# SNUCP/MKHE-KKLSS

Measured on AMD Instinct MI355X. Metric: mkckks_mulrelin_per_sec, higher is better.
Workload: dtype u64; 1 GPU; mkckks 4-party MulRelin (hoist + MulAndRelinHoisted + Rescale), PN15QP880 N=2^15, 14 Q + 2 P limbs; parties=4, params=PN15QP880, seed=1296779333, key_material=host

## Files before the change

### mkhe-kklss_amd/csrc/ntt_kernels.hip

```cpp
#include "ntt_kernels.h"
#include <stdexcept>
#include <cstdlib>
#include <mutex>
#ifndef MKHE_SB_MASK
#define MKHE_SB_MASK 1
#endif
#ifndef MKHE_TW_CHUNK
#define MKHE_TW_CHUNK 4
#endif

namespace mkhe {

typedef const __attribute__((address_space(1))) u64* gcptr;
typedef __attribute__((address_space(1))) u64* gptr;

template <int LOGN> struct Geo {
    static constexpr int N = 1 << LOGN;
    static constexpr int T = N / 32;
    static constexpr int BT = T < 64 ? 64 : T;
    static constexpr int LPB = BT / T;
    static constexpr int MIDTOP = (LOGN - 6) < 9 ? (LOGN - 6) : 9;
    static constexpr int MIDB = MIDTOP - 5;
    static constexpr bool HAS_MID = MIDTOP >= 5;
};
// ... 68 lines not shown
    if constexpr (!CROSS) lds_sync<false>();
}

__device__ __forceinline__ void bfly_fwd_cs(u64& U, u64& V, u64 ws, u64 q, u64 q2, u64 qs, u32 ninv) {
    u64 Tm = mont_mul_sdu(V, ws, qs, q, ninv);
    u64 u = csub(U, q2);
    U = u + Tm;
    V = u + (q2 - Tm);
}
__device__ __forceinline__ void bfly_fwd_nr(u64& U, u64& V, u64 ws, u64 qs, u32 ninv) {
    const i64 Tm = mont_mul_sd((i64)V, ws, qs, ninv);
    const i64 u = (i64)U;
    U = (u64)(u + Tm);
    V = (u64)(u - Tm);
}
__device__ __forceinline__ void bfly_inv(u64& U, u64& V, u64 ws, u64 q, u64 q2, u64 qs, u32 ninv) {
    u64 s = csub(U + V, q2);
    u64 d = U + q2 - V;
    U = s;
    V = mont_mul_sdu(d, ws, qs, q, ninv);
}

template <int B, int MODE>
__device__ __forceinline__ void stage(u64 (&x)[32], gcptr tw, u64 q, u64 q2, u64 qs, u32 ninv) {
    constexpr int NW = 16 >> B;
#ifdef MKHE_NO_CHUNK
    constexpr int CH = NW;
#else
    constexpr int CH = NW < MKHE_TW_CHUNK ? NW : MKHE_TW_CHUNK;
#endif
    constexpr int NCH = NW / CH;
    constexpr int BPC = 16 / NCH;
    u64 wc[CH], wn[CH];
#pragma unroll
    for (int k = 0; k < CH; ++k) wc[k] = tw[k];
#pragma unroll
    for (int c = 0; c < NCH; ++c) {
        if (c + 1 < NCH) {
#pragma unroll
            for (int k = 0; k < CH; ++k) wn[k] = tw[(c + 1) * CH + k];
        }
#pragma unroll
        for (int gg = 0; gg < BPC; ++gg) {
            const int g = c * BPC + gg;
            const int i0 = ((g >> B) << (B + 1)) | (g & ((1 << B) - 1));
            const int i1 = i0 | (1 << B);
            const u64 w = wc[(g >> B) - c * CH];
            if constexpr (MODE == 2) bfly_inv(x[i0], x[i1], w, q, q2, qs, ninv);
            else if constexpr (MODE == 1) bfly_fwd_nr(x[i0], x[i1], w, qs, ninv);
            else bfly_fwd_cs(x[i0], x[i1], w, q, q2, qs, ninv);
#ifndef MKHE_NO_SCHEDBAR
            if ((gg & MKHE_SB_MASK) == MKHE_SB_MASK) __builtin_amdgcn_sched_barrier(0);
#endif
        }
        if (c + 1 < NCH) {
#pragma unroll
            for (int k = 0; k < CH; ++k) wc[k] = wn[k];
        }
    }
    asm volatile("" ::: "memory");
}

template <int MODE>
__device__ __forceinline__ void phase(u64 (&x)[32], gcptr psi, int base, int prefix, int maxB, u64 q, u64 q2, u64 qs, u32 ninv) {
    if constexpr (MODE != 2) {
        if (maxB >= 4) stage<4, MODE>(x, psi + (base >> 4) + prefix, q, q2, qs, ninv);
        if (maxB >= 3) stage<3, MODE>(x, psi + (base >> 3) + (prefix << 1), q, q2, qs, ninv);
        if (maxB >= 2) stage<2, MODE>(x, psi + (base >> 2) + (prefix << 2), q, q2, qs, ninv);
        if (maxB >= 1) stage<1, MODE>(x, psi + (base >> 1) + (prefix << 3), q, q2, qs, ninv);
        if (maxB >= 0) stage<0, MODE>(x, psi + base + (prefix << 4), q, q2, qs, ninv);
    } else {
        if (maxB >= 0) stage<0, MODE>(x, psi + base + (prefix << 4), q, q2, qs, ninv);
        if (maxB >= 1) stage<1, MODE>(x, psi + (base >> 1) + (prefix << 3), q, q2, qs, ninv);
        if (maxB >= 2) stage<2, MODE>(x, psi + (base >> 2) + (prefix << 2), q, q2, qs, ninv);
        if (maxB >= 3) stage<3, MODE>(x, psi + (base >> 3) + (prefix << 1), q, q2, qs, ninv);
        if (maxB >= 4) stage<4, MODE>(x, psi + (base >> 4) + prefix, q, q2, qs, ninv);
    }
}

typedef const __attribute__((address_space(4))) NttBatch* kargptr;
__device__ __forceinline__ unsigned vi_parts_of(kargptr kb, int item) {
    return (((const __attribute__((address_space(4))) unsigned*)kb->vi_parts)[item >> 1] >> (16 * (item & 1))) & 0xffffu;
}
template <bool VI = false>
__device__ __forceinline__ int job_pointers(const NttBatch& b, int job, gcptr& src, gptr& dst, int& m, int& outer, int* pm = nullptr) {
    kargptr kb = (kargptr)__builtin_amdgcn_kernarg_segment_ptr();
    const int s = job / b.nouter;
    outer = job - s * b.nouter;
    m = kb->mod[s];
    if (VI && b.vi) {
        const int cnt = kb->vi_cnt[outer];
        const int k = s < b.vi_q ? 0 : (s - b.vi_q) / b.vi_np;
        const bool exists = k < cnt;
        const unsigned mem = kb->vi_mem[outer];
        const int item = (int)((mem >> (exists ? 8 * k : 0)) & 255u);
        const long off = (long)item * b.src_outer + (long)m * b.src_inner;
        src = (gcptr)(b.src + off);
        dst = (gptr)(b.dst + off);
        if (pm) *pm = s < b.vi_q ? -1 : k;
        if (!exists) return 0;
        if (s >= b.vi_q) return 1 + (int)(vi_parts_of(kb, item) & 255u);
        int n = kb->vi_extra[outer] != nullptr ? 1 : 0;
        for (int j = 0; j < cnt; ++j) n += 1 + (int)(vi_parts_of(kb, (mem >> (8 * j)) & 255u) & 255u);
        return n;
    }
    if (pm) *pm = -1;
    const int p = kb->pos[s];
    const u64* sbase = b.src; u64* dbase = b.dst;
    if (b.nitems > 0) {
        const int item = outer / b.outers_per_item;
        outer -= item * b.outers_per_item;
        sbase = kb->src_items[item]; dbase = kb->dst_items[item];
    }
    src = (gcptr)(sbase + (long)outer * b.src_outer + (long)(b.src_mapped ? m : p) * b.src_inner);
    dst = (gptr)(dbase + (long)outer * b.dst_outer + (long)(b.dst_mapped ? m : p) * b.dst_inner);
    return 1;
}
__device__ __forceinline__ long vi_member_offset(const NttBatch& b, int g, int k, int m, gcptr first) {
    kargptr kb = (kargptr)__builtin_amdgcn_kernarg_segment_ptr();
    if (k >= kb->vi_cnt[g]) return (long)(((u64)kb->vi_extra[g] - (u64)first) >> 3) + (long)m * b.src_inner;
    const unsigned mem = kb->vi_mem[g];
    return ((long)((mem >> (8 * k)) & 255u) - (long)(mem & 255u)) * b.src_outer;
}
__device__ __forceinline__ long vi_summand_offset(const NttBatch& b, int g, int pm, int k, int m, gcptr first) {
    kargptr kb = (kargptr)__builtin_amdgcn_kernarg_segment_ptr();
    const unsigned mem = kb->vi_mem[g];
    if (pm >= 0) {
        const int item = (int)((mem >> (8 * pm)) & 255u);
        return ((long)(vi_parts_of(kb, item) >> 8) + (k - 1) - (long)item) * b.src_outer;
    }
    const int cnt = kb->vi_cnt[g], item0 = (int)(mem & 255u);
    int kk = k;
    for (int j = 0; j < cnt; ++j) {
        const int item = (int)((mem >> (8 * j)) & 255u);
        const unsigned parts = vi_parts_of(kb, item);
        const int np_ = 1 + (int)(parts & 255u);
        if (kk < np_) return ((long)(kk == 0 ? item : (int)(parts >> 8) + kk - 1) - (long)item0) * b.src_outer;
        kk -= np_;
    }
    return (long)(((u64)kb->vi_extra[g] - (u64)first) >> 3) + (long)m * b.src_inner;
}

#ifdef MKHE_PHASE_TRACE
#define MKHE_STAMP(k) do { if (b.trace && (threadIdx.x & 63) == 0 && active) b.trace[((long)job * 16 + (threadIdx.x >> 6)) * 16 + (k)] = __builtin_amdgcn_s_memtime(); } while (0)
#else
#define MKHE_STAMP(k) do { } while (0)
#endif
template <int LOGN, int MODE, bool DEC>
__device__ __forceinline__ void ntt_fwd_job(const NttBatch& b, int job, bool active, u32* lds, int t) {
    using G = Geo<LOGN>;
#ifdef MKHE_PHASE_TRACE
    if (b.trace && (threadIdx.x & 63) == 0 && active) {
        u64* tw = b.trace + ((long)job * 16 + (threadIdx.x >> 6)) * 16;
        tw[12] = __builtin_amdgcn_s_memrealtime();
        tw[14] = __builtin_amdgcn_s_getreg((4 << 0) | (0 << 6) | (31 << 11));
    }
#endif
    MKHE_STAMP(0);
    gcptr src; gptr dst; int m, outer;
    const int half = b.split ? (job & 1) : 0;
    job_pointers(b, b.split ? (job >> 1) : job, src, dst, m, outer);
    src += half * G::N; dst += half * G::N;
    const int root = b.split ? 2 + half : 1;
    const Mod md = b.mods[m];
    const u64 q = md.q, q2 = md.q2;
    const u32 ninv = md.ninv32;
    gcptr psi = (gcptr)(b.psi + ((long)m * G::N << b.split));

    u64 x[32];
#pragma unroll
    for (int r = 0; r < 32; ++r) x[r] = src[posA<LOGN>(t, r)];
#ifdef MKHE_PHASE_TRACE
    if (b.trace) { asm volatile("s_waitcnt vmcnt(0)" ::: "memory"); MKHE_STAMP(1); }
#endif
    if constexpr (DEC) {
        int sm = m;
        if (b.reduce_src_mod_is_outer == 1) sm = outer;
        else if (b.reduce_src_mod_is_outer == 2) sm = ((kargptr)__builtin_amdgcn_kernarg_segment_ptr())->outer_mod[outer];
        const u64 qs = b.mods[sm].q << (b.src_lazy ? 2 : 0);
        if (qs > 4 * q) {
#pragma unroll
            for (int r = 0; r < 32; ++r) {
                if constexpr (MODE == 1) x[r] = (u64)mont_mul_sd((i64)x[r], md.r1s, md.qs, ninv);
                else x[r] = mont_mul_sdu(x[r], md.r1s, md.qs, q, ninv);
            }
        }
    }
#pragma unroll 1
    for (int ph = 0; ph < 3; ++ph) {
        int base = 16, prefix = 0, maxB = 4;
        if (ph == 1) { base = G::N >> 6; prefix = t >> 5; maxB = G::MIDB; }
        if (ph == 2) { base = G::N >> 1; prefix = t; }
        phase<MODE>(x, psi, base * root, prefix, maxB, q, q2, md.qs, ninv);
        MKHE_STAMP(2 + 2 * ph);
        if (ph == 0) {
            if constexpr (G::HAS_MID) {
                __syncthreads();
                exchange<LOGN, LA, LB, true>(x, lds, t);
            }
        } else if (ph == 1) exchange<LOGN, LB, LC, false>(x, lds, t);
        MKHE_STAMP(3 + 2 * ph);
    }
    if constexpr (MODE == 1) {
        if (!b.skip_norm) {
#pragma unroll
            for (int r = 0; r < 32; ++r) {
                const i64 y = mont_mul_sd((i64)x[r], md.r1s, md.qs, ninv);
                x[r] = (u64)(y + ((y >> 63) & (i64)q));
            }
        } else {
            const i64 bias = (i64)(q << 4);
#pragma unroll
            for (int r = 0; r < 32; ++r) x[r] = (u64)((i64)x[r] + bias);
        }
    } else {
#pragma unroll
        for (int r = 0; r < 32; ++r) x[r] = csub(csub(x[r], q2), q);
    }
    MKHE_STAMP(7);
    exchange<LOGN, LC, LB, false>(x, lds, t);
    MKHE_STAMP(8);
    if (active) {
#pragma unroll
// ... 82 lines not shown
        phase<2>(x, psi, base * root, prefix, maxB, q, q2, md.qs, ninv);
        if (ph == 0) exchange_xor<LOGN, LC, LB, false>(x, lds, t);
        else { if constexpr (G::HAS_MID) exchange_xor<LOGN, LB, LA, true>(x, lds, t); }
    }
    phase<2>(x, psi, 16 * root, 0, 3, q, q2, md.qs, ninv);
    const int ax = 6 * m + (b.split ? 2 + 2 * half : 0);
    const u64 ninvR = b.aux[ax], w1n = b.aux[ax + 1];
#pragma unroll
    for (int g = 0; g < 16; ++g) {
        u64 U = x[g], V = x[g + 16];
        u64 s = mont_mul_sdu(U + V, ninvR, md.qs, q, ninv);
        u64 d = mont_mul_sdu(U + q2 - V, w1n, md.qs, q, ninv);
        x[g] = (b.lazy_out | b.split) ? s : csub(s, q);
        x[g + 16] = (b.lazy_out | b.split) ? d : csub(d, q);
    }
    if (exists) {
#pragma unroll
        for (int r = 0; r < 32; ++r) dst[posA<LOGN>(t, r)] = x[r];
    }
    }
}

constexpr int SPLIT_THREADS = 256;
template <bool DEC>
__global__ void __launch_bounds__(SPLIT_THREADS) ntt_split_fwd_kernel(NttBatch b, int logN) {
    const int N = 1 << logN, H = N >> 1;
    gcptr src; gptr dst; int m, outer;
    job_pointers(b, blockIdx.y, src, dst, m, outer);
    const Mod md = b.mods[m];
    const u64 q = md.q, q2 = md.q2;
    const u32 ninv = md.ninv32;
    const u64 w = b.psi[(long)m * N + 1];
    bool red = false;
    if constexpr (DEC) {
        int sm = m;
        if (b.reduce_src_mod_is_outer == 1) sm = outer;
        else if (b.reduce_src_mod_is_outer == 2) sm = ((kargptr)__builtin_amdgcn_kernarg_segment_ptr())->outer_mod[outer];
        const u64 qs = b.mods[sm].q << (b.src_lazy ? 2 : 0);
        red = qs > 4 * q;
    }
    for (int j = blockIdx.x * SPLIT_THREADS + threadIdx.x; j < H; j += gridDim.x * SPLIT_THREADS) {
        u64 U = src[j], V = src[j + H];
        if (red) { U = mont_mul_sdu(U, md.r1s, md.qs, q, ninv); V = mont_mul_sdu(V, md.r1s, md.qs, q, ninv); }
        else U = csub(U, q2);
        const u64 Tm = mont_mul_sdu(V, w, md.qs, q, ninv);
        dst[j] = U + Tm;
        dst[j + H] = U + (q2 - Tm);
    }
}
__global__ void __launch_bounds__(SPLIT_THREADS) ntt_split_inv_kernel(NttBatch b, int logN) {
    const int N = 1 << logN, H = N >> 1;
    gcptr src; gptr dst; int m, outer;
    if (!job_pointers<true>(b, blockIdx.y, src, dst, m, outer)) return;
    const Mod md = b.mods[m];
    const u64 q = md.q, q2 = md.q2;
    const u32 ninv = md.ninv32;
    const u64 w = b.psi[(long)m * N + 1];
    for (int j = blockIdx.x * SPLIT_THREADS + threadIdx.x; j < H; j += gridDim.x * SPLIT_THREADS) {
        const u64 U = dst[j], V = dst[j + H];
        u64 s = csub(U + V, q2);
        u64 d = mont_mul_sdu(U + q2 - V, w, md.qs, q, ninv);
        if (!b.lazy_out) { s = csub(s, q); d = csub(d, q); }
        dst[j] = s;
        dst[j + H] = d;
    }
}
constexpr int SM_LOGM = 13, SM_M = 1 << SM_LOGM, SM_T = 1024, SM_E = SM_M / SM_T;
constexpr int SM_LDS_WORDS = SM_M + (SM_M >> 3);
__device__ __forceinline__ int sm_pad(int p) { return p + ((p >> 4) << 1); }

template <int LOGM> struct SmGeo { static constexpr int T = LOGM == 11 ? 256 : LOGM == 12 ? 512 : SM_T, E = (1 << LOGM) / T, LDSW = (1 << LOGM) + (1 << (LOGM - 3)); };
template <int S0, int NB, int LOGM>
__device__ __forceinline__ void sm_tw_load(gcptr psi, int root, int t, u64* tw) {
    constexpr int LGL = LOGM - S0 - NB, UPT = SmGeo<LOGM>::E >> NB, NE = 1 << NB;
#pragma unroll
    for (int k = 0; k < UPT; ++k) {
        const int high = (k * SmGeo<LOGM>::T + t) >> LGL;
#pragma unroll
        for (int i = 0; i < NB; ++i)
#pragma unroll
            for (int j = 0; j < (1 << i); ++j) tw[k * (NE - 1) + (1 << i) - 1 + j] = psi[(root << (S0 + i)) + (high << i) + j];
    }
}
template <int S0, int NB, bool FROM_G, bool TO_G, int MODE, int FIN, int LOGM = SM_LOGM, bool PRE = false>
__device__ __forceinline__ void sm_phase(gcptr gsrc, gptr gdst, u64* lds, gcptr psi, int root, int t, const Mod& md, u64 fin_c, int skip_norm,
                                         int nsum = 1, const long* sum_off = nullptr, const u64* tw = nullptr) {
    constexpr int LGL = LOGM - S0 - NB, GL = 1 << LGL, UPT = SmGeo<LOGM>::E >> NB, NE = 1 << NB;
    const u64 q = md.q, q2 = md.q2;
    const u32 ninv = md.ninv32;
#pragma unroll
    for (int k = 0; k < UPT; ++k) {
        const int u = k * SmGeo<LOGM>::T + t;
        const int low = u & (GL - 1), high = u >> LGL;
        const int p = (high << (LGL + NB)) | low;
        u64 x[NE];
#pragma unroll
        for (int a = 0; a < NE; ++a) x[a] = FROM_G ? gsrc[p + a * GL] : lds[sm_pad(p + a * GL)];
        if constexpr (FROM_G && MODE == 2) {
#pragma unroll
            for (int k = 1; k < VI_SUMS; ++k)
                if (k < nsum) {
#pragma unroll
                    for (int a = 0; a < NE; ++a) x[a] = csub(x[a] + gsrc[sum_off[k] + p + a * GL], q);
                }
        }
#pragma unroll
        for (int ii = 0; ii < NB; ++ii) {
            const int i = MODE == 2 ? NB - 1 - ii : ii;
            const int half = 1 << (NB - 1 - i);
#pragma unroll
            for (int a = 0; a < NE; ++a) {
                if (a & half) continue;
                const u64 w = PRE ? tw[k * (NE - 1) + (1 << i) - 1 + (a >> (NB - i))] : psi[(root << (S0 + i)) + (high << i) + (a >> (NB - i))];
                if constexpr (MODE == 2) bfly_inv(x[a], x[a + half], w, q, q2, md.qs, ninv);
                else if constexpr (MODE == 1) bfly_fwd_nr(x[a], x[a + half], w, md.qs, ninv);
                else bfly_fwd_cs(x[a], x[a + half], w, q, q2, md.qs, ninv);
            }
        }
#pragma unroll
        for (int a = 0; a < NE; ++a) {
            u64 v = x[a];
            if constexpr (FIN == 1) {
                if constexpr (MODE == 1) {
                    if (!skip_norm) { const i64 y = mont_mul_sd((i64)v, md.r1s, md.qs, ninv); v = (u64)(y + ((y >> 63) & (i64)q)); }
                    else v = (u64)((i64)v + (i64)(q << 4));
                } else v = csub(csub(v, q2), q);
            } else if constexpr (FIN == 2) v = mont_mul_sdu(v, fin_c, md.qs, q, ninv);
            if constexpr (TO_G) gdst[p + a * GL] = v; else lds[sm_pad(p + a * GL)] = v;
        }
    }
}

template <int MODE, int LOGM = SM_LOGM>
__global__ void __launch_bounds__(SmGeo<LOGM>::T) ntt_fwd_lds_kernel(NttBatch b, int d) {
    extern __shared__ __attribute__((aligned(16))) u64 sm_lds[];
    constexpr int M = 1 << LOGM;
    const int job = blockIdx.x, part = job & ((1 << d) - 1), t = threadIdx.x;
    gcptr src; gptr dst; int m, outer;
    job_pointers(b, job >> d, src, dst, m, outer);
    src += part * M; dst += part * M;
    const int root = (1 << d) + part;
    const Mod md = b.mods[m];
    gcptr psi = (gcptr)(b.psi + ((long)m * M << d));
    if constexpr (LOGM <= 12) {
        constexpr int NBL = LOGM == 12 ? 3 : 2, NL = (SmGeo<LOGM>::E >> NBL) * ((1 << NBL) - 1);
        u64 t0[7], t1[7], t2[7], t3[NL];
        sm_tw_load<0, 3, LOGM>(psi, root, t, t0); sm_tw_load<3, 3, LOGM>(psi, root, t, t1);
        sm_tw_load<6, 3, LOGM>(psi, root, t, t2); sm_tw_load<9, NBL, LOGM>(psi, root, t, t3);
        sm_phase<0, 3, true, false, MODE, 0, LOGM, true>(src, dst, sm_lds, psi, root, t, md, 0, 0, 1, nullptr, t0);
        __syncthreads();
        sm_phase<3, 3, false, false, MODE, 0, LOGM, true>(src, dst, sm_lds, psi, root, t, md, 0, 0, 1, nullptr, t1);
        __syncthreads();
        sm_phase<6, 3, false, false, MODE, 0, LOGM, true>(src, dst, sm_lds, psi, root, t, md, 0, 0, 1, nullptr, t2);
        __syncthreads();
        sm_phase<9, NBL, false, true, MODE, 1, LOGM, true>(src, dst, sm_lds, psi, root, t, md, 0, b.skip_norm, 1, nullptr, t3);
    } else {
        sm_phase<0, 3, true, false, MODE, 0, LOGM>(src, dst, sm_lds, psi, root, t, md, 0, 0);
        __syncthreads();
        sm_phase<3, 3, false, false, MODE, 0, LOGM>(src, dst, sm_lds, psi, root, t, md, 0, 0);
        __syncthreads();
        sm_phase<6, 3, false, false, MODE, 0, LOGM>(src, dst, sm_lds, psi, root, t, md, 0, 0);
        __syncthreads();
        sm_phase<9, 3, false, false, MODE, 0, LOGM>(src, dst, sm_lds, psi, root, t, md, 0, 0);
        __syncthreads();
        sm_phase<12, 1, false, true, MODE, 1, LOGM>(src, dst, sm_lds, psi, root, t, md, 0, b.skip_norm);
    }
}

template <int LOGM>
__global__ void __launch_bounds__(SmGeo<LOGM>::T) ntt_inv_ldsS_kernel(NttBatch b, int d) {
    extern __shared__ __attribute__((aligned(16))) u64 sm_lds[];
    constexpr int M = 1 << LOGM;
    const int job = blockIdx.x, part = job & ((1 << d) - 1), t = threadIdx.x;
    gcptr src; gptr dst; int m, outer;
    int pm = -1;
    const int nsum = job_pointers<true>(b, job >> d, src, dst, m, outer, &pm);
    if (nsum == 0) return;
    long sum_off[VI_SUMS] = {};
#pragma unroll
    for (int k = 1; k < VI_SUMS; ++k) if (k < nsum) sum_off[k] = vi_summand_offset(b, outer, pm, k, m, src);
    src += part * M; dst += part * M;
    const int root = (1 << d) + part;
    const Mod md = b.mods[m];
    gcptr psi = (gcptr)(b.psi + ((long)m * M << d));
    const u64 ninvR = b.aux[6 * m];
    constexpr int NBL = LOGM == 12 ? 3 : 2, NL = (SmGeo<LOGM>::E >> NBL) * ((1 << NBL) - 1);
    u64 t0[7], t1[7], t2[7], t3[NL];
    sm_tw_load<9, NBL, LOGM>(psi, root, t, t3); sm_tw_load<6, 3, LOGM>(psi, root, t, t2);
    sm_tw_load<3, 3, LOGM>(psi, root, t, t1); sm_tw_load<0, 3, LOGM>(psi, root, t, t0);
    sm_phase<9, NBL, true, false, 2, 0, LOGM, true>(src, dst, sm_lds, psi, root, t, md, 0, 0, nsum, sum_off, t3);
    __syncthreads();
    sm_phase<6, 3, false, false, 2, 0, LOGM, true>(src, dst, sm_lds, psi, root, t, md, 0, 0, 1, nullptr, t2);
    __syncthreads();
    sm_phase<3, 3, false, false, 2, 0, LOGM, true>(src, dst, sm_lds, psi, root, t, md, 0, 0, 1, nullptr, t1);
    __syncthreads();
    sm_phase<0, 3, false, true, 2, 2, LOGM, true>(src, dst, sm_lds, psi, root, t, md, ninvR, 0, 1, nullptr, t0);
}

__global__ void __launch_bounds__(SPLIT_THREADS) ntt_pass_fwd_kernel(NttBatch b, int logN, int L) {
    const int N = 1 << logN, G = N >> (L + 1);
    gcptr src; gptr dst; int m, outer;
    job_pointers(b, blockIdx.y, src, dst, m, outer);
    const Mod md = b.mods[m];
    const u64 q = md.q, q2 = md.q2;
    const u32 ninv = md.ninv32;
    for (int j = blockIdx.x * SPLIT_THREADS + threadIdx.x; j < (N >> 1); j += gridDim.x * SPLIT_THREADS) {
        const int blk = j >> (logN - L - 1), off = j - blk * G, i0 = blk * 2 * G + off;
        const u64 w = b.psi[(long)m * N + (1 << L) + blk];
        const u64 U = csub(dst[i0], q2), V = dst[i0 + G];
        const u64 Tm = mont_mul_sdu(V, w, md.qs, q, ninv);
        dst[i0] = U + Tm;
        dst[i0 + G] = U + (q2 - Tm);
    }
}
__global__ void __launch_bounds__(SPLIT_THREADS) ntt_pass_inv_kernel(NttBatch b, int logN, int L) {
    const int N = 1 << logN, G = N >> (L + 1);
    gcptr src; gptr dst; int m, outer;
    if (!job_pointers<true>(b, blockIdx.y, src, dst, m, outer)) return;
    const Mod md = b.mods[m];
    const u64 q = md.q, q2 = md.q2;
    const u32 ninv = md.ninv32;
    for (int j = blockIdx.x * SPLIT_THREADS + threadIdx.x; j < (N >> 1); j += gridDim.x * SPLIT_THREADS) {
        const int blk = j >> (logN - L - 1), off = j - blk * G, i0 = blk * 2 * G + off;
        const u64 w = b.psi[(long)m * N + (1 << L) + blk];
        const u64 U = dst[i0], V = dst[i0 + G];
        dst[i0] = csub(U + V, q2);
        dst[i0 + G] = mont_mul_sdu(U + q2 - V, w, md.qs, q, ninv);
    }
}

template <bool DEC>
__global__ void __launch_bounds__(SPLIT_THREADS) ntt_pass4_fwd_kernel(NttBatch b, int logN) {
    const int N = 1 << logN, Q = N >> 2;
    gcptr src; gptr dst; int m, outer;
    job_pointers(b, blockIdx.y, src, dst, m, outer);
    const Mod md = b.mods[m];
    const u64 q = md.q, q2 = md.q2;
    const u32 ninv = md.ninv32;
    const u64 w1 = b.psi[(long)m * N + 1], w2 = b.psi[(long)m * N + 2], w3 = b.psi[(long)m * N + 3];
    bool red = false;
    if constexpr (DEC) {
        int sm = m;
        if (b.reduce_src_mod_is_outer == 1) sm = outer;
        else if (b.reduce_src_mod_is_outer == 2) sm = ((kargptr)__builtin_amdgcn_kernarg_segment_ptr())->outer_mod[outer];
        const u64 qs = b.mods[sm].q << (b.src_lazy ? 2 : 0);
        red = qs > 4 * q;
    }
    for (int j = blockIdx.x * SPLIT_THREADS + threadIdx.x; j < Q; j += gridDim.x * SPLIT_THREADS) {
        u64 a0 = src[j], a1 = src[j + Q], a2 = src[j + 2 * Q], a3 = src[j + 3 * Q];
        if (red) {
            a0 = mont_mul_sdu(a0, md.r1s, md.qs, q, ninv); a1 = mont_mul_sdu(a1, md.r1s, md.qs, q, ninv);
            a2 = mont_mul_sdu(a2, md.r1s, md.qs, q, ninv); a3 = mont_mul_sdu(a3, md.r1s, md.qs, q, ninv);
        } else { a0 = csub(a0, q2); a1 = csub(a1, q2); }
        u64 T = mont_mul_sdu(a2, w1, md.qs, q, ninv);
        const u64 b0 = a0 + T, b2 = a0 + (q2 - T);
        T = mont_mul_sdu(a3, w1, md.qs, q, ninv);
        const u64 b1 = a1 + T, b3 = a1 + (q2 - T);
        u64 u = csub(b0, q2);
        T = mont_mul_sdu(b1, w2, md.qs, q, ninv);
        dst[j] = u + T; dst[j + Q] = u + (q2 - T);
        u = csub(b2, q2);
        T = mont_mul_sdu(b3, w3, md.qs, q, ninv);
        dst[j + 2 * Q] = u + T; dst[j + 3 * Q] = u + (q2 - T);
    }
}
__global__ void __launch_bounds__(SPLIT_THREADS) ntt_pass4_inv_kernel(NttBatch b, int logN) {
    const int N = 1 << logN, Q = N >> 2;
    gcptr src; gptr dst; int m, outer;
    if (!job_pointers<true>(b, blockIdx.y, src, dst, m, outer)) return;
    const Mod md = b.mods[m];
    const u64 q = md.q, q2 = md.q2;
    const u32 ninv = md.ninv32;
    const u64 w1 = b.psi[(long)m * N + 1], w2 = b.psi[(long)m * N + 2], w3 = b.psi[(long)m * N + 3];
    for (int j = blockIdx.x * SPLIT_THREADS + threadIdx.x; j < Q; j += gridDim.x * SPLIT_THREADS) {
        const u64 a0 = dst[j], a1 = dst[j + Q], a2 = dst[j + 2 * Q], a3 = dst[j + 3 * Q];
        const u64 s0 = csub(a0 + a1, q2), d0 = mont_mul_sdu(a0 + q2 - a1, w2, md.qs, q, ninv);
        const u64 s1 = csub(a2 + a3, q2), d1 = mont_mul_sdu(a2 + q2 - a3, w3, md.qs, q, ninv);
        u64 r0 = csub(s0 + s1, q2), r2 = mont_mul_sdu(s0 + q2 - s1, w1, md.qs, q, ninv);
        u64 r1 = csub(d0 + d1, q2), r3 = mont_mul_sdu(d0 + q2 - d1, w1, md.qs, q, ninv);
// ... 59 lines not shown
    long moff[VI_MAX] = {};
    const int ns = b.sum_in_cross ? nsum : 1;
#pragma unroll
    for (int k = 1; k < VI_MAX; ++k) if (k < ns) moff[k] = vi_member_offset(b, outer, k, m, src);
    auto gs = [&](u64& x, u64& y, u64 tw) {
        const u64 s_ = csub(x + y, q2), d_ = mont_mul_sdu(x + q2 - y, tw, md.qs, q, ninv);
        x = s_; y = d_;
    };
    for (int j = blockIdx.x * SPLIT_THREADS + threadIdx.x; j < E; j += gridDim.x * SPLIT_THREADS) {
        u64 a[8];
#pragma unroll
        for (int k = 0; k < 8; ++k) a[k] = dst[j + k * E];
#pragma unroll
        for (int mm = 1; mm < VI_MAX; ++mm)
            if (mm < ns) {
#pragma unroll
                for (int k = 0; k < 8; ++k) a[k] = csub(a[k] + dst[moff[mm] + j + k * E], q2);
            }
#pragma unroll
        for (int c = 0; c < 4; ++c) gs(a[2 * c], a[2 * c + 1], w[4 + c]);
#pragma unroll
        for (int h = 0; h < 2; ++h)
#pragma unroll
            for (int k = 0; k < 2; ++k) gs(a[4 * h + k], a[4 * h + k + 2], w[2 + h]);
#pragma unroll
        for (int k = 0; k < 4; ++k) gs(a[k], a[k + 4], w[1]);
#pragma unroll
        for (int k = 0; k < 8; ++k) dst[j + k * E] = b.lazy_out ? a[k] : csub(a[k], q);
    }
}

template <int NG, int MODE, bool INV>
__device__ __forceinline__ void extf_body(const ExtFusedArgs& a, u64* lds, const Mod& md, int m, int part, int v) {
    constexpr int LOGM = 11, M = 1 << LOGM, TALL = NG * 256, CPT = M / TALL;
    const int g = threadIdx.x >> 8, t = threadIdx.x & 255;
    const int d = a.logN - LOGM, root = (1 << d) + part;
    gcptr psi = (gcptr)(a.psi + (long)m * a.N);
    u64* region = lds + g * SmGeo<LOGM>::LDSW;
    constexpr int NL = (SmGeo<LOGM>::E >> 2) * 3;
    u64 t0[7], t1[7], t2[7], t3[NL];
    sm_tw_load<0, 3, LOGM>(psi, root, t, t0); sm_tw_load<3, 3, LOGM>(psi, root, t, t1);
    sm_tw_load<6, 3, LOGM>(psi, root, t, t2); sm_tw_load<9, 2, LOGM>(psi, root, t, t3);
    const u64 q = md.q, q2 = md.q2;
    const u32 ninv = md.ninv32;
    const long limb = (long)m * a.N + (long)part * M;
    const int nk = a.nk[v];
    gcptr st = (gcptr)a.stage[v];
    gcptr k0 = (gcptr)a.bg[v][0], k1 = (gcptr)a.bg[v][1];
    u64 acc0[CPT], acc1[CPT];
#pragma unroll
    for (int j = 0; j < CPT; ++j) { acc0[j] = 0; acc1[j] = 0; }
    constexpr bool PF = true, PFS = true;
    static_assert(NG == 1 || NG == 2, "three and four groups (768 / 1024 threads) spill and were measured slower");
    static_assert(!INV || NG == 2, "the inverse sub-transforms are the work of two groups");
    u64 xn[8];
    if constexpr (PFS) {
        if (g < a.nb) {
#pragma unroll
            for (int e = 0; e < 8; ++e) xn[e] = st[(long)g * a.digit_stride + limb + t + 256 * e];
        }
    }
    for (int r = 0; r * NG < a.nb; ++r) {
        const int dg = r * NG + g;
        const bool active = dg < a.nb;
        gcptr src = st + (long)dg * a.digit_stride + limb;
        u64 kv0[PF ? NG : 1][CPT], kv1[PF ? NG : 1][CPT];
        if constexpr (PF) {
#pragma unroll
            for (int dd = 0; dd < NG; ++dd) {
                const int dig = r * NG + dd;
                const long ko = (long)(dig < a.nb ? dig : 0) * a.digit_stride + limb;
#pragma unroll
                for (int j = 0; j < CPT; ++j) {
                    const int pos = (int)threadIdx.x + j * TALL;
                    kv0[dd][j] = k0[ko + pos];
                    kv1[dd][j] = nk > 1 ? k1[ko + pos] : 0;
                }
            }
        }
        if constexpr (PFS) {
            if (active) {
#pragma unroll
                for (int e = 0; e < 8; ++e) region[sm_pad(t + 256 * e)] = xn[e];
                sm_phase<0, 3, false, false, MODE, 0, LOGM, true>(src, nullptr, region, psi, root, t, md, 0, 0, 1, nullptr, t0);
            }
            if (dg + NG < a.nb) {
#pragma unroll
                for (int e = 0; e < 8; ++e) xn[e] = st[(long)(dg + NG) * a.digit_stride + limb + t + 256 * e];
            }
        } else if (active) sm_phase<0, 3, true, false, MODE, 0, LOGM, true>(src, nullptr, region, psi, root, t, md, 0, 0, 1, nullptr, t0);
        __syncthreads();
        if (active) sm_phase<3, 3, false, false, MODE, 0, LOGM, true>(src, nullptr, region, psi, root, t, md, 0, 0, 1, nullptr, t1);
        __syncthreads();
        if (active) sm_phase<6, 3, false, false, MODE, 0, LOGM, true>(src, nullptr, region, psi, root, t, md, 0, 0, 1, nullptr, t2);
        __syncthreads();
        if (active) sm_phase<9, 2, false, false, MODE, 1, LOGM, true>(src, nullptr, region, psi, root, t, md, 0, 1, 1, nullptr, t3);
        __syncthreads();
#pragma unroll
        for (int dd = 0; dd < NG; ++dd) {
            const int dig = r * NG + dd;
            if (dig < a.nb) {
                const long ko = (long)dig * a.digit_stride + limb;
#pragma unroll
                for (int j = 0; j < CPT; ++j) {
                    const int pos = (int)threadIdx.x + j * TALL;
                    const u64 h = lds[dd * SmGeo<LOGM>::LDSW + sm_pad(pos)];
                    const u64 g0 = PF ? kv0[PF ? dd : 0][j] : k0[ko + pos];
                    acc0[j] = csub(acc0[j] + mont_mul_lazy(g0, h, q, ninv), q2);
                    if (nk > 1) { const u64 g1 = PF ? kv1[PF ? dd : 0][j] : k1[ko + pos]; acc1[j] = csub(acc1[j] + mont_mul_lazy(g1, h, q, ninv), q2); }
                }
            }
        }
        __syncthreads();
    }
    if constexpr (INV) {
#pragma unroll
        for (int j = 0; j < CPT; ++j) {
            const int pos = (int)threadIdx.x + j * TALL;
            lds[sm_pad(pos)] = csub(acc0[j], q);
            if (nk > 1) lds[SmGeo<LOGM>::LDSW + sm_pad(pos)] = csub(acc1[j], q);
        }
        __syncthreads();
        const bool work = g < nk;
        gcptr psii = (gcptr)(a.psiinv + (long)m * a.N);
        const u64 ninvR = a.aux[6 * m];
        u64 i0[7], i1[7], i2[7], i3[NL];
        if (work) {
            sm_tw_load<9, 2, LOGM>(psii, root, t, i3); sm_tw_load<6, 3, LOGM>(psii, root, t, i2);
            sm_tw_load<3, 3, LOGM>(psii, root, t, i1); sm_tw_load<0, 3, LOGM>(psii, root, t, i0);
            sm_phase<9, 2, false, false, 2, 0, LOGM, true>(nullptr, nullptr, region, psii, root, t, md, 0, 0, 1, nullptr, i3);
        }
        __syncthreads();
        if (work) sm_phase<6, 3, false, false, 2, 0, LOGM, true>(nullptr, nullptr, region, psii, root, t, md, 0, 0, 1, nullptr, i2);
        __syncthreads();
        if (work) sm_phase<3, 3, false, false, 2, 0, LOGM, true>(nullptr, nullptr, region, psii, root, t, md, 0, 0, 1, nullptr, i1);
        __syncthreads();
        if (work) sm_phase<0, 3, false, true, 2, 2, LOGM, true>(nullptr, (gptr)(a.out[v][g] + limb), region, psii, root, t, md, ninvR, 0, 1, nullptr, i0);
    } else {
    u64* o0 = a.out[v][0] + limb; u64* o1 = a.out[v][1];
#pragma unroll
    for (int j = 0; j < CPT; ++j) {
        const int pos = (int)threadIdx.x + j * TALL;
        o0[pos] = csub(acc0[j], q);
        if (nk > 1) o1[limb + pos] = csub(acc1[j], q);
    }
    }
}
template <int NG, bool INV>
__global__ void __launch_bounds__(NG * 256) ext_fused_lds_kernel(ExtFusedArgs a) {
    extern __shared__ __attribute__((aligned(16))) u64 sm_lds[];
    const int part = blockIdx.x, m = a.map[blockIdx.y], v = blockIdx.z;
    const Mod md = a.mods[m];
    if ((a.small_mask >> m) & 1) extf_body<NG, 1, INV>(a, sm_lds, md, m, part, v);
    else extf_body<NG, 0, INV>(a, sm_lds, md, m, part, v);
}

static NttBatch in_place_of_dst(const NttBatch& b) {
    NttBatch c = b;
    c.src = b.dst; c.src_outer = b.dst_outer; c.src_inner = b.dst_inner; c.src_mapped = b.dst_mapped;
    for (int i = 0; i < NTT_MAX_ITEMS; ++i) c.src_items[i] = b.dst_items[i];
    c.reduce_in = 0; c.split = 1;
    return c;
}

namespace {
struct LaunchState { std::mutex mu; int resident[64] = {}; bool attr[64] = {}; };
int current_device() { int dev = 0; (void)hipGetDevice(&dev); return dev & 63; }
}
static int resident_blocks(const void* fn, int threads, size_t lds) {
#ifdef MKHE_SWITCHES
    if (const char* e = getenv("MKHE_NTT_GRID")) { if (e[0] == 'f') return 1 << 30; }
#endif
    int dev = 0, cus = 256, per = 1;
    (void)hipGetDevice(&dev);
    (void)hipDeviceGetAttribute(&cus, hipDeviceAttributeMultiprocessorCount, dev);
    if (hipOccupancyMaxActiveBlocksPerMultiprocessor(&per, fn, threads, lds) != hipSuccess || per < 1) per = 1;
    return cus * per;
}
template <int LOGN, int MODE, bool DEC> static void launch_fwd_t(const NttBatch& b, hipStream_t st) {
    using G = Geo<LOGN>;
    static LaunchState ls;
    const size_t lds = (size_t)G::LPB * lds_words<LOGN>() * sizeof(u32);
    int resident;
    {
        const int dev = current_device();
        std::lock_guard<std::mutex> g(ls.mu);
        if (!ls.attr[dev]) { (void)hipFuncSetAttribute((const void*)ntt_fwd_kernel<LOGN, MODE, DEC>, hipFuncAttributeMaxDynamicSharedMemorySize, (int)lds); ls.attr[dev] = true; }
        if (!ls.resident[dev]) ls.resident[dev] = resident_blocks((const void*)ntt_fwd_kernel<LOGN, MODE, DEC>, G::BT, lds);
        resident = ls.resident[dev];
    }
    const int need = (((b.nslots * b.nouter) << b.split) + G::LPB - 1) / G::LPB;
    const int blocks = need < resident ? need : resident;
    hipLaunchKernelGGL((ntt_fwd_kernel<LOGN, MODE, DEC>), dim3(blocks), dim3(G::BT), lds, st, b);
}
template <int LOGN, bool VI> static void launch_inv_tv(const NttBatch& b, hipStream_t st) {
    using G = Geo<LOGN>;
    static LaunchState ls;
    const size_t lds = (size_t)G::LPB * lds_words<LOGN>() * sizeof(u32);
    int resident;
    {
        const int dev = current_device();
        std::lock_guard<std::mutex> g(ls.mu);
        if (!ls.attr[dev]) { (void)hipFuncSetAttribute((const void*)ntt_inv_kernel<LOGN, VI>, hipFuncAttributeMaxDynamicSharedMemorySize, (int)lds); ls.attr[dev] = true; }
        if (!ls.resident[dev]) ls.resident[dev] = resident_blocks((const void*)ntt_inv_kernel<LOGN, VI>, G::BT, lds);
        resident = ls.resident[dev];
    }
    const int need = (((b.nslots * b.nouter) << b.split) + G::LPB - 1) / G::LPB;
    const int blocks = need < resident ? need : resident;
    hipLaunchKernelGGL((ntt_inv_kernel<LOGN, VI>), dim3(blocks), dim3(G::BT), lds, st, b);
}
template <int LOGN> static void launch_inv_t(const NttBatch& b, hipStream_t st) {
    if (b.vi) launch_inv_tv<LOGN, true>(b, st); else launch_inv_tv<LOGN, false>(b, st);
}

template <int MODE, bool DEC> static void launch_fwd_mode(int logN, const NttBatch& b, hipStream_t st) {
    switch (logN) {
        case 10: launch_fwd_t<10, MODE, DEC>(b, st); break;
        case 11: launch_fwd_t<11, MODE, DEC>(b, st); break;
        case 12: launch_fwd_t<12, MODE, DEC>(b, st); break;
        case 13: launch_fwd_t<13, MODE, DEC>(b, st); break;
// ... 212 lines not shown
```

Before: 1350 MulRelin/s.

## Batch summand loads in inverse LDS NTT and compute offsets lane-parallel

The inverse small-LDS NTT kernel now gathers and sums all virtual-item summands up front through a new sm_sum_load helper. It loads summands in blocks of two so several global loads are in flight before the additions, instead of interleaving load and add inside the first butterfly phase. Summand offsets are computed once per wave, with each lane handling one summand index and results broadcast via readlane, replacing a serial per-summand loop. The kernel also gains a minimum-occupancy launch bound for LOGM 12. The cost is more registers for the preloaded values, which may reduce occupancy.

```diff
diff --git a/mkhe-kklss_amd/csrc/ntt_kernels.hip b/mkhe-kklss_amd/csrc/ntt_kernels.hip
--- a/mkhe-kklss_amd/csrc/ntt_kernels.hip
+++ b/mkhe-kklss_amd/csrc/ntt_kernels.hip
@@ -174,7 +174,7 @@
 __device__ __forceinline__ unsigned vi_parts_of(kargptr kb, int item) {
     return (((const __attribute__((address_space(4))) unsigned*)kb->vi_parts)[item >> 1] >> (16 * (item & 1))) & 0xffffu;
 }
-template <bool VI = false>
+template <bool VI = false, bool COUNT = true>
 __device__ __forceinline__ int job_pointers(const NttBatch& b, int job, gcptr& src, gptr& dst, int& m, int& outer, int* pm = nullptr) {
     kargptr kb = (kargptr)__builtin_amdgcn_kernarg_segment_ptr();
     const int s = job / b.nouter;
@@ -191,6 +191,7 @@
         dst = (gptr)(b.dst + off);
         if (pm) *pm = s < b.vi_q ? -1 : k;
         if (!exists) return 0;
+        if (!COUNT) return 1;
         if (s >= b.vi_q) return 1 + (int)(vi_parts_of(kb, item) & 255u);
         int n = kb->vi_extra[outer] != nullptr ? 1 : 0;
         for (int j = 0; j < cnt; ++j) n += 1 + (int)(vi_parts_of(kb, (mem >> (8 * j)) & 255u) & 255u);
@@ -231,6 +232,38 @@
         kk -= np_;
     }
     return (long)(((u64)kb->vi_extra[g] - (u64)first) >> 3) + (long)m * b.src_inner;
+}
+__device__ __forceinline__ int vi_summand_offsets(const NttBatch& b, int g, int pm, int m, gcptr first, int t, long (&off)[VI_SUMS]) {
+    kargptr kb = (kargptr)__builtin_amdgcn_kernarg_segment_ptr();
+#pragma unroll
+    for (int kk = 0; kk < VI_SUMS; ++kk) off[kk] = 0;
+    if (!b.vi) return 1;
+    const u64* const xp = kb->vi_extra[g];
+    const unsigned mem = kb->vi_mem[g] >> (pm >= 0 ? 8 * pm : 0);
+    const int cnt = pm >= 0 ? 1 : kb->vi_cnt[g], item0 = (int)(mem & 255u);
+    const long extra = (long)(((u64)xp - (u64)first) >> 3) + (long)m * b.src_inner;
+    int item[VI_MAX], np_[VI_MAX], base[VI_MAX];
+#pragma unroll
+    for (int j = 0; j < VI_MAX; ++j) {
+        item[j] = j < cnt ? (int)((mem >> (8 * j)) & 255u) : item0;
+        const unsigned parts = vi_parts_of(kb, item[j]);
+        np_[j] = j < cnt ? 1 + (int)(parts & 255u) : 0;
+        base[j] = (int)(parts >> 8);
+    }
+    const int k = t & 63;
+    int idx = item0, s = 0;
+#pragma unroll
+    for (int j = 0; j < VI_MAX; ++j) {
+        const int r = k - s;
+        idx = r >= 0 && r < np_[j] ? (r == 0 ? item[j] : base[j] + r - 1) : idx;
+        s += np_[j];
+    }
+    const int nsum = s + (pm < 0 && xp != nullptr ? 1 : 0);
+    const long o = k >= nsum ? 0 : k >= s ? extra : (long)(idx - item0) * b.src_outer;
+#pragma unroll
+    for (int kk = 1; kk < VI_SUMS; ++kk)
+        off[kk] = (long)(((u64)(u32)__builtin_amdgcn_readlane((int)((u64)o >> 32), kk) << 32) | (u32)__builtin_amdgcn_readlane((int)(u64)o, kk));
+    return nsum;
 }
 
 #ifdef MKHE_PHASE_TRACE
@@ -479,9 +512,44 @@
             for (int j = 0; j < (1 << i); ++j) tw[k * (NE - 1) + (1 << i) - 1 + j] = psi[(root << (S0 + i)) + (high << i) + j];
     }
 }
+constexpr int SM_SUM_BLOCK = 2;
+template <int S0, int NB, int LOGM>
+__device__ __forceinline__ void sm_sum_load(gcptr gsrc, int t, u64 q, int nsum, const long* sum_off, u64* xs) {
+    constexpr int LGL = LOGM - S0 - NB, GL = 1 << LGL, UPT = SmGeo<LOGM>::E >> NB, NE = 1 << NB, E = SmGeo<LOGM>::E;
+    int p[UPT];
+#pragma unroll
+    for (int k = 0; k < UPT; ++k) {
+        const int u = k * SmGeo<LOGM>::T + t;
+        p[k] = ((u >> LGL) << (LGL + NB)) | (u & (GL - 1));
+#pragma unroll
+        for (int a = 0; a < NE; ++a) xs[k * NE + a] = gsrc[p[k] + a * GL];
+    }
+#pragma unroll
+    for (int k0 = 1; k0 < VI_SUMS; k0 += SM_SUM_BLOCK) {
+        if (k0 < nsum) {
+            constexpr int B = SM_SUM_BLOCK;
+            u64 y[B][E];
+#pragma unroll
+            for (int j = 0; j < B; ++j) {
+                if (k0 + j >= VI_SUMS) continue;
+#pragma unroll
+                for (int k = 0; k < UPT; ++k)
+#pragma unroll
+                    for (int a = 0; a < NE; ++a) y[j][k * NE + a] = gsrc[sum_off[k0 + j] + p[k] + a * GL];
+            }
+#pragma unroll
+            for (int j = 0; j < B; ++j) {
+                if (k0 + j >= VI_SUMS) continue;
+                const u64 keep = k0 + j < nsum ? ~0ull : 0ull;
+#pragma unroll
+                for (int e = 0; e < E; ++e) xs[e] = csub(xs[e] + (y[j][e] & keep), q);
+            }
+        }
+    }
+}
 template <int S0, int NB, bool FROM_G, bool TO_G, int MODE, int FIN, int LOGM = SM_LOGM, bool PRE = false>
 __device__ __forceinline__ void sm_phase(gcptr gsrc, gptr gdst, u64* lds, gcptr psi, int root, int t, const Mod& md, u64 fin_c, int skip_norm,
-                                         int nsum = 1, const long* sum_off = nullptr, const u64* tw = nullptr) {
+                                         const u64* tw = nullptr, const u64* xin = nullptr) {
     constexpr int LGL = LOGM - S0 - NB, GL = 1 << LGL, UPT = SmGeo<LOGM>::E >> NB, NE = 1 << NB;
     const u64 q = md.q, q2 = md.q2;
     const u32 ninv = md.ninv32;
@@ -492,15 +560,7 @@
         const int p = (high << (LGL + NB)) | low;
         u64 x[NE];
 #pragma unroll
-        for (int a = 0; a < NE; ++a) x[a] = FROM_G ? gsrc[p + a * GL] : lds[sm_pad(p + a * GL)];
-        if constexpr (FROM_G && MODE == 2) {
-#pragma unroll
-            for (int k = 1; k < VI_SUMS; ++k)
-                if (k < nsum) {
-#pragma unroll
-                    for (int a = 0; a < NE; ++a) x[a] = csub(x[a] + gsrc[sum_off[k] + p + a * GL], q);
-                }
-        }
+        for (int a = 0; a < NE; ++a) x[a] = !FROM_G ? lds[sm_pad(p + a * GL)] : xin ? xin[k * NE + a] : gsrc[p + a * GL];
 #pragma unroll
         for (int ii = 0; ii < NB; ++ii) {
             const int i = MODE == 2 ? NB - 1 - ii : ii;
@@ -544,13 +604,13 @@
         u64 t0[7], t1[7], t2[7], t3[NL];
         sm_tw_load<0, 3, LOGM>(psi, root, t, t0); sm_tw_load<3, 3, LOGM>(psi, root, t, t1);
         sm_tw_load<6, 3, LOGM>(psi, root, t, t2); sm_tw_load<9, NBL, LOGM>(psi, root, t, t3);
-        sm_phase<0, 3, true, false, MODE, 0, LOGM, true>(src, dst, sm_lds, psi, root, t, md, 0, 0, 1, nullptr, t0);
-        __syncthreads();
-        sm_phase<3, 3, false, false, MODE, 0, LOGM, true>(src, dst, sm_lds, psi, root, t, md, 0, 0, 1, nullptr, t1);
-        __syncthreads();
-        sm_phase<6, 3, false, false, MODE, 0, LOGM, true>(src, dst, sm_lds, psi, root, t, md, 0, 0, 1, nullptr, t2);
-        __syncthreads();
-        sm_phase<9, NBL, false, true, MODE, 1, LOGM, true>(src, dst, sm_lds, psi, root, t, md, 0, b.skip_norm, 1, nullptr, t3);
+        sm_phase<0, 3, true, false, MODE, 0, LOGM, true>(src, dst, sm_lds, psi, root, t, md, 0, 0, t0);
+        __syncthreads();
+        sm_phase<3, 3, false, false, MODE, 0, LOGM, true>(src, dst, sm_lds, psi, root, t, md, 0, 0, t1);
+        __syncthreads();
+        sm_phase<6, 3, false, false, MODE, 0, LOGM, true>(src, dst, sm_lds, psi, root, t, md, 0, 0, t2);
+        __syncthreads();
+        sm_phase<9, NBL, false, true, MODE, 1, LOGM, true>(src, dst, sm_lds, psi, root, t, md, 0, b.skip_norm, t3);
     } else {
         sm_phase<0, 3, true, false, MODE, 0, LOGM>(src, dst, sm_lds, psi, root, t, md, 0, 0);
         __syncthreads();
@@ -565,33 +625,32 @@
 }
 
 template <int LOGM>
-__global__ void __launch_bounds__(SmGeo<LOGM>::T) ntt_inv_ldsS_kernel(NttBatch b, int d) {
+__global__ void __launch_bounds__(SmGeo<LOGM>::T, LOGM == 12 ? 6 : 1) ntt_inv_ldsS_kernel(NttBatch b, int d) {
     extern __shared__ __attribute__((aligned(16))) u64 sm_lds[];
     constexpr int M = 1 << LOGM;
     const int job = blockIdx.x, part = job & ((1 << d) - 1), t = threadIdx.x;
     gcptr src; gptr dst; int m, outer;
     int pm = -1;
-    const int nsum = job_pointers<true>(b, job >> d, src, dst, m, outer, &pm);
-    if (nsum == 0) return;
-    long sum_off[VI_SUMS] = {};
-#pragma unroll
-    for (int k = 1; k < VI_SUMS; ++k) if (k < nsum) sum_off[k] = vi_summand_offset(b, outer, pm, k, m, src);
+    if (!job_pointers<true, false>(b, job >> d, src, dst, m, outer, &pm)) return;
+    long sum_off[VI_SUMS];
+    const int nsum = vi_summand_offsets(b, outer, pm, m, src, t, sum_off);
     src += part * M; dst += part * M;
     const int root = (1 << d) + part;
     const Mod md = b.mods[m];
     gcptr psi = (gcptr)(b.psi + ((long)m * M << d));
     const u64 ninvR = b.aux[6 * m];
     constexpr int NBL = LOGM == 12 ? 3 : 2, NL = (SmGeo<LOGM>::E >> NBL) * ((1 << NBL) - 1);
-    u64 t0[7], t1[7], t2[7], t3[NL];
-    sm_tw_load<9, NBL, LOGM>(psi, root, t, t3); sm_tw_load<6, 3, LOGM>(psi, root, t, t2);
-    sm_tw_load<3, 3, LOGM>(psi, root, t, t1); sm_tw_load<0, 3, LOGM>(psi, root, t, t0);
-    sm_phase<9, NBL, true, false, 2, 0, LOGM, true>(src, dst, sm_lds, psi, root, t, md, 0, 0, nsum, sum_off, t3);
+    u64 t0[7], t1[7], t2[7], t3[NL], xs[SmGeo<LOGM>::E];
+    sm_tw_load<9, NBL, LOGM>(psi, root, t, t3);
+    sm_sum_load<9, NBL, LOGM>(src, t, md.q, nsum, sum_off, xs);
+    sm_tw_load<6, 3, LOGM>(psi, root, t, t2); sm_tw_load<3, 3, LOGM>(psi, root, t, t1); sm_tw_load<0, 3, LOGM>(psi, root, t, t0);
+    sm_phase<9, NBL, true, false, 2, 0, LOGM, true>(src, dst, sm_lds, psi, root, t, md, 0, 0, t3, xs);
     __syncthreads();
-    sm_phase<6, 3, false, false, 2, 0, LOGM, true>(src, dst, sm_lds, psi, root, t, md, 0, 0, 1, nullptr, t2);
+    sm_phase<6, 3, false, false, 2, 0, LOGM, true>(src, dst, sm_lds, psi, root, t, md, 0, 0, t2);
     __syncthreads();
-    sm_phase<3, 3, false, false, 2, 0, LOGM, true>(src, dst, sm_lds, psi, root, t, md, 0, 0, 1, nullptr, t1);
+    sm_phase<3, 3, false, false, 2, 0, LOGM, true>(src, dst, sm_lds, psi, root, t, md, 0, 0, t1);
     __syncthreads();
-    sm_phase<0, 3, false, true, 2, 2, LOGM, true>(src, dst, sm_lds, psi, root, t, md, ninvR, 0, 1, nullptr, t0);
+    sm_phase<0, 3, false, true, 2, 2, LOGM, true>(src, dst, sm_lds, psi, root, t, md, ninvR, 0, t0);
 }
 
 __global__ void __launch_bounds__(SPLIT_THREADS) ntt_pass_fwd_kernel(NttBatch b, int logN, int L) {
@@ -817,19 +876,19 @@
             if (active) {
 #pragma unroll
                 for (int e = 0; e < 8; ++e) region[sm_pad(t + 256 * e)] = xn[e];
-                sm_phase<0, 3, false, false, MODE, 0, LOGM, true>(src, nullptr, region, psi, root, t, md, 0, 0, 1, nullptr, t0);
+                sm_phase<0, 3, false, false, MODE, 0, LOGM, true>(src, nullptr, region, psi, root, t, md, 0, 0, t0);
             }
             if (dg + NG < a.nb) {
 #pragma unroll
                 for (int e = 0; e < 8; ++e) xn[e] = st[(long)(dg + NG) * a.digit_stride + limb + t + 256 * e];
             }
-        } else if (active) sm_phase<0, 3, true, false, MODE, 0, LOGM, true>(src, nullptr, region, psi, root, t, md, 0, 0, 1, nullptr, t0);
-        __syncthreads();
-        if (active) sm_phase<3, 3, false, false, MODE, 0, LOGM, true>(src, nullptr, region, psi, root, t, md, 0, 0, 1, nullptr, t1);
-        __syncthreads();
-        if (active) sm_phase<6, 3, false, false, MODE, 0, LOGM, true>(src, nullptr, region, psi, root, t, md, 0, 0, 1, nullptr, t2);
-        __syncthreads();
-        if (active) sm_phase<9, 2, false, false, MODE, 1, LOGM, true>(src, nullptr, region, psi, root, t, md, 0, 1, 1, nullptr, t3);
+        } else if (active) sm_phase<0, 3, true, false, MODE, 0, LOGM, true>(src, nullptr, region, psi, root, t, md, 0, 0, t0);
+        __syncthreads();
+        if (active) sm_phase<3, 3, false, false, MODE, 0, LOGM, true>(src, nullptr, region, psi, root, t, md, 0, 0, t1);
+        __syncthreads();
+        if (active) sm_phase<6, 3, false, false, MODE, 0, LOGM, true>(src, nullptr, region, psi, root, t, md, 0, 0, t2);
+        __syncthreads();
+        if (active) sm_phase<9, 2, false, false, MODE, 1, LOGM, true>(src, nullptr, region, psi, root, t, md, 0, 1, t3);
         __syncthreads();
 #pragma unroll
         for (int dd = 0; dd < NG; ++dd) {
@@ -863,14 +922,14 @@
         if (work) {
             sm_tw_load<9, 2, LOGM>(psii, root, t, i3); sm_tw_load<6, 3, LOGM>(psii, root, t, i2);
             sm_tw_load<3, 3, LOGM>(psii, root, t, i1); sm_tw_load<0, 3, LOGM>(psii, root, t, i0);
-            sm_phase<9, 2, false, false, 2, 0, LOGM, true>(nullptr, nullptr, region, psii, root, t, md, 0, 0, 1, nullptr, i3);
-        }
-        __syncthreads();
-        if (work) sm_phase<6, 3, false, false, 2, 0, LOGM, true>(nullptr, nullptr, region, psii, root, t, md, 0, 0, 1, nullptr, i2);
-        __syncthreads();
-        if (work) sm_phase<3, 3, false, false, 2, 0, LOGM, true>(nullptr, nullptr, region, psii, root, t, md, 0, 0, 1, nullptr, i1);
-        __syncthreads();
-        if (work) sm_phase<0, 3, false, true, 2, 2, LOGM, true>(nullptr, (gptr)(a.out[v][g] + limb), region, psii, root, t, md, ninvR, 0, 1, nullptr, i0);
+            sm_phase<9, 2, false, false, 2, 0, LOGM, true>(nullptr, nullptr, region, psii, root, t, md, 0, 0, i3);
+        }
+        __syncthreads();
+        if (work) sm_phase<6, 3, false, false, 2, 0, LOGM, true>(nullptr, nullptr, region, psii, root, t, md, 0, 0, i2);
+        __syncthreads();
+        if (work) sm_phase<3, 3, false, false, 2, 0, LOGM, true>(nullptr, nullptr, region, psii, root, t, md, 0, 0, i1);
+        __syncthreads();
+        if (work) sm_phase<0, 3, false, true, 2, 2, LOGM, true>(nullptr, (gptr)(a.out[v][g] + limb), region, psii, root, t, md, ninvR, 0, i0);
     } else {
     u64* o0 = a.out[v][0] + limb; u64* o1 = a.out[v][1];
 #pragma unroll
```

Result: no change. 1351 MulRelin/s (median of 3 runs) (+0.1%).
